# asharakeh/pod_compare

Hardware: AMD Instinct MI355X
Metric: images/sec (BayesOD+MC-dropout, 1280x720) (higher is better)
Workload: dtype f32 (convolutions: every fp32 product from 2-way f16 splits of the power-of-two-scaled fp32 operands, 3 partial products, fp32 accumulate; closer to fp64 than the fp32 MFMA: profiles/r05_f16_split_numerics.txt)

## Files before the change

### include/pod_mi355x.h

```cpp
#ifndef POD_MI355X_H
#define POD_MI355X_H

#include <stddef.h>
#include <stdint.h>

#ifdef __cplusplus
extern "C" {
#endif

#define POD_ABI_VERSION 18
#define POD_MAX_LEVELS 8
#define POD_MAX_CLASSES 16
#define POD_MAX_RUNS 64
#define POD_MAX_TOPK 2048
#define POD_MAX_PROP_SAMPLES 1024
#define POD_MAX_CLS_SAMPLES 64
#define POD_MAX_CANDIDATES 8192
#define POD_MAX_DETECTIONS 128
#define POD_COCO_MAX_IOU 16
#define POD_COCO_MAX_REC 128
#define POD_COCO_MAX_AREA 4
#define POD_COCO_MAX_MAXDET 4
#define POD_COCO_MAX_KEEP 128
#define POD_COCO_LDS_GT 64
// ... 248 lines not shown
    const float* cov;
    const float* probs;
    const float* colours;
    const int32_t* count;
    float* out;
    int32_t* n_out;
    int32_t max_n, box_stride, cov_stride, prob_stride, n_probs, colour_mode, colour_stride;
    int32_t cov_pairing;
    float colour[4];
    int32_t frame_h, frame_w;
    float scale, alpha;
} PodVisList;

typedef struct PodVisFrame {
    const uint8_t* src;
    int64_t sy, sx, sc;
    int32_t src_h, src_w, bgr, bilinear;
    int32_t frame_h, frame_w, out_h, out_w;
    uint8_t* dst;
    float scale, stroke;
    const float* inst[2];
    const int32_t* n_inst[2];
    const float* labels;
    const uint8_t* atlas;
    int32_t n_labels, reserved;
} PodVisFrame;

int pod_vis_layout(const PodVisList* lists, int32_t n_lists, pod_stream_t stream);
int pod_vis_render(const PodVisFrame* frames, int32_t n_frames, pod_stream_t stream);


#define POD_C1_RELU 1
#define POD_C1_RESIDUAL_UP2 2
int64_t pod_conv1x1_filter_split_bytes(int32_t Cout, int32_t Cin);
int pod_conv1x1_filter_split(const float* weight, void* Ws, int32_t Cout, int32_t Cin, pod_stream_t stream);
int pod_reduce_partials(const float* partials, int32_t n_splits, int64_t split_stride, const float* bias, const float* residual, float* y,
                        int64_t n, int32_t Cout, int32_t relu, float* out_amax, pod_stream_t stream);
int pod_conv1x1_split(const float* x, float* y, const void* Ws, const float* bias, const float* residual, int32_t H_out, int32_t W_out,
                      int32_t H_in, int32_t W_in, int32_t stride, int32_t Cin, int32_t Cout, int32_t flags, int32_t n_splits, float* partials,
                      int32_t waves, const float* in_amax, float* out_amax, pod_stream_t stream);

typedef struct PodWorkspace {
    const float* anchors;
    float* mean_cls;  float* mean_cls_var;  float* mean_delta;  float* mean_reg_var;
    uint64_t* cand_keys;  int32_t* cand_count;  uint64_t* maybe_bits;
    uint64_t* sel_keys;   int32_t* sel_count;
    uint64_t* cat_keys;   int32_t* cat_level;
    float* probs_dense;
    int32_t* n_total;     int32_t* cand_anchor_idx;  int32_t* cand_level;  int32_t* cand_class;
    float* cand_score;    float* cand_probs;  float* cand_delta;  float* cand_reg_var;  float* cand_anchor;
    float* cand_run_delta;
    float* boxes;  float* cov;
    int32_t* keep;  int32_t* n_keep;  void* nms_scratch;
    float* m_boxes;  float* m_cov;  float* m_scores;  int32_t* m_classes;  float* m_probs;
    int32_t n_capacity;  int32_t reserved;
} PodWorkspace;

#define POD_MODE_STANDARD_NMS 0
#define POD_MODE_BAYES_OD 1
#define POD_MODE_ANCHOR_STATISTICS 2

int pod_run_image(const PodConfig* cfg, const PodLevel* levels, const PodWorkspace* ws, int32_t mode,
                  int32_t box_merge_mode, int32_t cls_merge_mode, int32_t image_h, int32_t image_w,
                  int32_t out_h, int32_t out_w, const PodDetections* out, pod_stream_t stream);
int pod_run_image_part(const PodConfig* cfg, const PodLevel* levels, const PodWorkspace* ws, int32_t mode,
                  int32_t box_merge_mode, int32_t cls_merge_mode, int32_t image_h, int32_t image_w,
// ... 7 lines not shown
```

### pod_compare_amd/conv1x1.py

```python
from typing import Optional

import torch

from . import amax, hip


class Conv1x1:

    def __init__(self, weight: torch.Tensor, bias: Optional[torch.Tensor], stride: int = 1):
        assert weight.is_cuda and weight.dtype == torch.float32 and weight.dim() == 4 and tuple(weight.shape[2:]) == (1, 1)
        self.K, self.C, self.stride = int(weight.shape[0]), int(weight.shape[1]), int(stride)
        if self.C % 16 or self.K % 64 or self.stride not in (1, 2):
            raise ValueError("pod_conv1x1_split: Cin %% 16 == 0, Cout %% 64 == 0, stride 1 or 2 required, got Cin=%d Cout=%d stride=%d" % (self.C, self.K, self.stride))
        self.Ws = torch.empty(2 * self.K * self.C + 8, dtype=torch.int16, device=weight.device)
        hip.check(hip.load().pod_conv1x1_filter_split(weight.detach().reshape(self.K, self.C).contiguous().data_ptr(), self.Ws.data_ptr(), self.K, self.C,
                                                      hip.current_stream()), "pod_conv1x1_filter_split")
        self.bias = None if bias is None else bias.detach().to(torch.float32).contiguous().clone()

    @staticmethod
    def eligible(conv: Optional[torch.nn.Conv2d]) -> bool:
        return (conv is not None and tuple(conv.kernel_size) == (1, 1) and tuple(conv.padding) == (0, 0) and conv.groups == 1
                and tuple(conv.dilation) == (1, 1) and conv.stride[0] == conv.stride[1] and conv.stride[0] in (1, 2)
                and conv.in_channels % 16 == 0 and conv.out_channels % 64 == 0)

    def out_hw(self, h: int, w: int):
        return ((h - 1) // self.stride + 1, (w - 1) // self.stride + 1)

    def splits_for(self, p_out: int, simds: int = 1024) -> int:
        tiles = ((p_out + 63) // 64) * (self.K // 64)
        nks = self.C // 16
        out_mb = p_out * self.K * 4 / 1e6
        step = 0.38
        best, best_t = 1, (nks // self.auto_waves(tiles, nks)) * step
        for s in (2, 4, 8, 16):
            if nks % s or nks // s < 4 or tiles * s > simds:
                continue
            t = (nks // s // self.auto_waves(tiles * s, nks // s)) * step + 3.0 + (s + 1) * out_mb / 4.0
            if t < best_t:
                best, best_t = s, t
        return best

    @staticmethod
    def auto_waves(tiles: int, per_split: int) -> int:
        waves = 1
        while waves < 4 and per_split % (waves * 4) == 0 and per_split // (waves * 2) >= 8 and tiles * waves * 2 <= 1024:
            waves *= 2
        return waves

    def __call__(self, x: torch.Tensor, h: int, w: int, relu: bool = False, residual: Optional[torch.Tensor] = None,
                 n_splits: Optional[int] = None, waves: int = 0, out: Optional[torch.Tensor] = None, residual_up2: bool = False) -> torch.Tensor:
        assert x.is_cuda and x.dtype == torch.float32 and x.is_contiguous() and tuple(x.shape) == (h * w, self.C)
        ho, wo = self.out_hw(h, w)
        y = torch.empty((ho * wo, self.K), dtype=torch.float32, device=x.device) if out is None else out
        assert y.is_contiguous() and tuple(y.shape) == (ho * wo, self.K) and y.dtype == torch.float32
        s = self.splits_for(ho * wo) if n_splits is None else int(n_splits)
        if residual is not None and residual_up2:
            hr, wr = (ho + 1) // 2, (wo + 1) // 2
            assert residual.is_contiguous() and tuple(residual.shape) == (hr * wr, self.K) and residual.dtype == torch.float32
            if s > 1:
                residual = residual.view(hr, wr, self.K).repeat_interleave(2, 0).repeat_interleave(2, 1)[:ho, :wo].reshape(ho * wo, self.K).contiguous()
                residual_up2 = False
        else:
            residual_up2 = False
        if residual is not None and not residual_up2:
            assert residual.is_contiguous() and tuple(residual.shape) == tuple(y.shape) and residual.dtype == torch.float32
        partials = torch.empty((s, ho * wo, self.K), dtype=torch.float32, device=x.device) if s > 1 else None
        hip.check(hip.load().pod_conv1x1_split(x.data_ptr(), y.data_ptr(), self.Ws.data_ptr(), hip.ptr(self.bias), hip.ptr(residual), ho, wo, h, w, self.stride,
                                               self.C, self.K, (1 if relu else 0) | (2 if residual_up2 else 0), s, hip.ptr(partials), int(waves), amax.of(x).data_ptr(), amax.produced(y).data_ptr(),
                                               hip.current_stream()), "pod_conv1x1_split")
        return y


class Stem7x7:

    def __init__(self, weight: torch.Tensor, bias: Optional[torch.Tensor]):
        assert weight.is_cuda and weight.dtype == torch.float32 and tuple(weight.shape) == (64, 3, 7, 7)
        self.Ws = torch.empty(2 * 64 * 192 + 8, dtype=torch.int16, device=weight.device)
        self._bounds = {}
        hip.check(hip.load().pod_stem7x7_filter_split(weight.detach().contiguous().data_ptr(), self.Ws.data_ptr(), hip.current_stream()), "pod_stem7x7_filter_split")
        self.bias = None if bias is None else bias.detach().to(torch.float32).contiguous().clone()

    @staticmethod
    def eligible(conv: Optional[torch.nn.Conv2d]) -> bool:
        return (conv is not None and tuple(conv.weight.shape) == (64, 3, 7, 7) and tuple(conv.stride) == (2, 2) and tuple(conv.padding) == (3, 3)
                and conv.groups == 1 and tuple(conv.dilation) == (1, 1))

    def __call__(self, x: torch.Tensor, relu: bool = True, mean: Optional[torch.Tensor] = None, std: Optional[torch.Tensor] = None,
                 padded_hw: Optional[tuple] = None):
        assert x.is_cuda and x.dtype in (torch.float32, torch.uint8) and x.is_contiguous() and x.numel() == 3 * x.shape[-2] * x.shape[-1]
        hi, wi = int(x.shape[-2]), int(x.shape[-1])
        h, w = (hi, wi) if padded_hw is None else (int(padded_hw[0]), int(padded_hw[1]))
        assert (mean is None) == (std is None) and h >= hi and w >= wi
        if mean is not None:
            assert mean.is_cuda and std.is_cuda and mean.dtype == std.dtype == torch.float32 and mean.numel() == std.numel() == 3 and mean.is_contiguous() and std.is_contiguous()
        ho, wo = (h - 1) // 2 + 1, (w - 1) // 2 + 1
        y = torch.empty((ho * wo, 64), dtype=torch.float32, device=x.device)
        bound = self._input_bound(x, mean, std)
        hip.check(hip.load().pod_stem7x7_split(x.data_ptr(), 1 if x.dtype == torch.uint8 else 0, hi, wi, hip.ptr(mean), hip.ptr(std), y.data_ptr(), self.Ws.data_ptr(),
                                               hip.ptr(self.bias), h, w, 1 if relu else 0, bound.data_ptr(), amax.produced(y).data_ptr(),
                                               hip.current_stream()), "pod_stem7x7_split")
        return y, ho, wo
# ... 53 lines not shown
```

### pod_compare_amd/csrc/k13_conv1x1_split.hip

```cpp
#include "pod_wino.h"

#ifdef POD_C1_TRACE
static __device__ long long g_c1_trace[8192 * 4];
static __device__ long long g_c1_cycles[8192 * 4];
#define C1_STAMP(k)                                                                                   \
    do {                                                                                              \
        const unsigned wg_ = blockIdx.y * gridDim.x + blockIdx.x;                                     \
        if (threadIdx.x == 0 && wg_ < 8192) {                                                         \
            g_c1_trace[wg_ * 4 + (k)] = wall_clock64();                                               \
            g_c1_cycles[wg_ * 4 + (k)] = clock64();                                                   \
        }                                                                                             \
    } while (0)
#else
#define C1_STAMP(k)
#endif

namespace pod {

typedef uint32_t c1_u32x4 __attribute__((ext_vector_type(4)));
constexpr int C1_KS_U16 = 2 * 2 * 256;
constexpr int C1_TOP = 14;

struct C1Params {
    const float* x;
// ... 160 lines not shown
            }
#pragma unroll
            for (int cb = 0; cb < NCB; ++cb)
#pragma unroll
                for (int q = 0; q < 4; ++q)
                    r[cb][q] = (k0 + 32 * cb + 8 * q < P.Cout) ? *reinterpret_cast<const f32x4*>(res + re0 + 32 * cb + 8 * q) : f32x4{0.f, 0.f, 0.f, 0.f};
        }
#pragma unroll
        for (int cb = 0; cb < NCB; ++cb) {
#pragma unroll
            for (int q = 0; q < 4; ++q) {
                const int k = k0 + 32 * cb + 8 * q;
                if (k >= P.Cout) continue;
                f32x4 v = f32x4{acc[cb][pb][4 * q], acc[cb][pb][4 * q + 1], acc[cb][pb][4 * q + 2], acc[cb][pb][4 * q + 3]};
                v = __builtin_elementwise_fma(v, inv, final_pass && bias ? *reinterpret_cast<const f32x4*>(bias + k) : f32x4{0.f, 0.f, 0.f, 0.f});
                if (final_pass) {
                    if (res) v += r[cb][q];
                    if (P.relu) {
                        v.x = fmaxf(v.x, 0.f); v.y = fmaxf(v.y, 0.f); v.z = fmaxf(v.z, 0.f); v.w = fmaxf(v.w, 0.f);
                    }
                    lmax = fmaxf(fmaxf(lmax, fmaxf(fabsf(v.x), fabsf(v.y))), fmaxf(fabsf(v.z), fabsf(v.w)));
                }
                if (!(POD_C1_ELIM & 8) || v.x == 12345.678f) *reinterpret_cast<f32x4*>(yo + e0 + 32 * cb + 8 * q) = v;
            }
        }
    }
    if (final_pass && P.out_amax) wino_publish_amax(P.out_amax, lmax);
#ifdef POD_C1_TRACE
    __builtin_amdgcn_s_waitcnt(0);
    C1_STAMP(3);
#endif
}

__device__ __forceinline__ void c1_epilogue(const C1Params& P, float* const lds_o, f32x16 (&acc)[2][2], int tp, int tc, int lane, int i32, int h, float sx) {
    constexpr int NCB = 2;
    const float inv1 = wino_pow2_inverse(sx) * wino_pow2_inverse(wino_pow2_scale(*reinterpret_cast<const float*>(P.Ws + (int64_t)P.Cout * P.Cin * 2), C1_TOP));
    const f32x4 inv = f32x4{inv1, inv1, inv1, inv1};
    float lmax = 0.0f;
    float* __restrict__ const yo = P.y + (int64_t)blockIdx.y * P.split_stride;
    const float* __restrict__ const res = P.residual;
    const bool final_pass = P.split_stride == 0;
    const int oc = lane & 15, op = lane >> 4;
    const int gp0 = tp * 64 + op;
    const int64_t e0 = (int64_t)gp0 * P.Cout + tc * 64 + 4 * oc;
    f32x4 r[16];
    if (final_pass && res && P.res_up2) {
        int oy = gp0 / P.W_out, ox = gp0 - oy * P.W_out;
#pragma unroll
        for (int j = 0; j < 16; ++j) {
            r[j] = (gp0 + 4 * j < P.P_out) ? *reinterpret_cast<const f32x4*>(res + ((int64_t)(oy >> 1) * P.W_res + (ox >> 1)) * P.Cout + tc * 64 + 4 * oc)
                                           : f32x4{0.f, 0.f, 0.f, 0.f};
            ox += 4;
            while (ox >= P.W_out) {
                ox -= P.W_out;
                ++oy;
            }
        }
    } else if (final_pass && res) {
#pragma unroll
        for (int j = 0; j < 16; ++j) r[j] = (gp0 + 4 * j < P.P_out) ? *reinterpret_cast<const f32x4*>(res + e0 + (int64_t)(4 * j) * P.Cout) : f32x4{0.f, 0.f, 0.f, 0.f};
    }
    f32x4 b4 = f32x4{0.f, 0.f, 0.f, 0.f};
    if (final_pass && P.bias) b4 = *reinterpret_cast<const f32x4*>(P.bias + tc * 64 + 4 * oc);
#pragma unroll
    for (int pb = 0; pb < 2; ++pb)
#pragma unroll
        for (int cb = 0; cb < NCB; ++cb)
#pragma unroll
            for (int q = 0; q < 4; ++q) {
                const int pix = 32 * pb + i32, c = 8 * cb + 2 * q + h;
                *reinterpret_cast<f32x4*>(lds_o + pix * 64 + 4 * (c ^ (i32 & 15))) =
                    f32x4{acc[cb][pb][4 * q], acc[cb][pb][4 * q + 1], acc[cb][pb][4 * q + 2], acc[cb][pb][4 * q + 3]};
            }
#pragma unroll
    for (int j = 0; j < 16; ++j) {
        const int pix = 4 * j + op;
        f32x4 v = __builtin_elementwise_fma(*reinterpret_cast<const f32x4*>(lds_o + pix * 64 + 4 * (oc ^ (pix & 15))), inv, b4);
        if (final_pass) {
            if (res) v += r[j];
            if (P.relu) {
                v.x = fmaxf(v.x, 0.f); v.y = fmaxf(v.y, 0.f); v.z = fmaxf(v.z, 0.f); v.w = fmaxf(v.w, 0.f);
            }
        }
        if (gp0 + 4 * j < P.P_out) {
            *reinterpret_cast<f32x4*>(yo + e0 + (int64_t)(4 * j) * P.Cout) = v;
            lmax = fmaxf(fmaxf(lmax, fmaxf(fabsf(v.x), fabsf(v.y))), fmaxf(fabsf(v.z), fabsf(v.w)));
        }
    }
    if (final_pass && P.out_amax) wino_publish_amax(P.out_amax, lmax);
}

template <int NCB, int WAVES>
__global__ void __launch_bounds__(64 * WAVES, WAVES > 1 ? 1 : 2) k_conv1x1_split_lds(const C1Params P) {
    __shared__ __attribute__((aligned(16))) float lds_all[WAVES][2][64 * 32];
    const int wave = threadIdx.x >> 6;
    float (*const lds_a)[64 * 32] = lds_all[wave];
    const int lane = threadIdx.x & 63, i32 = lane & 31, h = lane >> 5;
    const int xcd = blockIdx.x & 7, wi = (int)(blockIdx.x >> 3);
    const int tp = (wi / P.n_ct) * 8 + xcd, tc = wi % P.n_ct;
    if (tp >= P.n_pt) return;
    C1_STAMP(0);
    const int nks_all = P.Cin >> 4, nks = P.ks_per_split / WAVES, ks0 = (int)blockIdx.y * P.ks_per_split + wave * nks;
    int32_t soff[8];
#pragma unroll
    for (int j = 0; j < 8; ++j) {
        const int pl = 8 * j + (lane >> 3), p = tp * 64 + pl;
        const int q = p < P.P_out ? p : 0;
        int pin = q;
        if (P.stride != 1) {
            const int oy = q / P.W_out, ox = q - oy * P.W_out;
            pin = (P.stride * oy) * P.W_in + P.stride * ox;
        }
        soff[j] = pin * P.Cin + ks0 * 16 + 4 * ((lane & 7) ^ ((pl >> 1) & 7));
    }
    const float* __restrict__ const xg = P.x;
    const int key = (i32 >> 1) & 7;
    const uint16_t* __restrict__ const wa = P.Ws + ((int64_t)(tc * NCB) * nks_all + ks0) * C1_KS_U16 + (h * 32 + i32) * 8;
    const int64_t w_cb = (int64_t)nks_all * C1_KS_U16;
    const float sx = __builtin_bit_cast(float, __builtin_amdgcn_readfirstlane(__builtin_bit_cast(int, wino_pow2_scale(wino_read_amax(P.in_amax), C1_TOP))));

    f32x16 acc[NCB][2];
#pragma unroll
// ... 76 lines not shown
    for (int j0 = 0; j0 < nks; j0 += 6) trip(trip, c1_ic<0>{}, j0);
    C1_STAMP(2);

    if constexpr (WAVES > 1) {
        if (wave > 0) {
            float* o = &lds_a[0][0];
#pragma unroll
            for (int cb = 0; cb < NCB; ++cb)
#pragma unroll
                for (int pb = 0; pb < 2; ++pb)
#pragma unroll
                    for (int r = 0; r < 16; ++r) o[((cb * 2 + pb) * 16 + r) * 64 + lane] = acc[cb][pb][r];
        }
        __syncthreads();
        if (wave > 0) return;
#pragma unroll
        for (int w = 1; w < WAVES; ++w) {
            const float* o = &lds_all[w][0][0];
#pragma unroll
            for (int cb = 0; cb < NCB; ++cb)
#pragma unroll
                for (int pb = 0; pb < 2; ++pb)
#pragma unroll
                    for (int r = 0; r < 16; ++r) acc[cb][pb][r] += o[((cb * 2 + pb) * 16 + r) * 64 + lane];
        }
    }
    c1_epilogue(P, &lds_a[0][0], acc, tp, tc, lane, i32, h, sx);
#ifdef POD_C1_TRACE
    __builtin_amdgcn_s_waitcnt(0);
    C1_STAMP(3);
#endif
}

__global__ void __launch_bounds__(256) k_conv1x1_reduce(const float* __restrict__ partials, int32_t n_splits, int64_t split_stride, const float* __restrict__ bias,
                                                        const float* __restrict__ residual, float* __restrict__ y, int64_t n4, int32_t Cout, int32_t relu,
                                                        float* __restrict__ out_amax) {
    const int64_t stride = (int64_t)gridDim.x * blockDim.x;
    float lmax = 0.0f;
    for (int64_t i = (int64_t)blockIdx.x * blockDim.x + threadIdx.x; i < n4; i += stride) {
        f32x4 v = *reinterpret_cast<const f32x4*>(partials + 4 * i);
        for (int s = 1; s < n_splits; ++s) v += *reinterpret_cast<const f32x4*>(partials + (int64_t)s * split_stride + 4 * i);
        if (bias) v += *reinterpret_cast<const f32x4*>(bias + (int)((4 * i) % Cout));
        if (residual) v += *reinterpret_cast<const f32x4*>(residual + 4 * i);
        if (relu) {
            v.x = fmaxf(v.x, 0.f); v.y = fmaxf(v.y, 0.f); v.z = fmaxf(v.z, 0.f); v.w = fmaxf(v.w, 0.f);
        }
        *reinterpret_cast<f32x4*>(y + 4 * i) = v;
        lmax = fmaxf(fmaxf(lmax, fmaxf(fabsf(v.x), fabsf(v.y))), fmaxf(fabsf(v.z), fabsf(v.w)));
    }
    if (out_amax) wino_publish_amax_block(out_amax, lmax);
}

}

extern "C" int64_t pod_conv1x1_filter_split_bytes(int32_t Cout, int32_t Cin) {
    if (Cout < 32 || (Cout & 31) != 0 || Cin < 16 || (Cin & 15) != 0) return 0;
    return (int64_t)Cout * Cin * 4 + 16;
}

extern "C" int pod_conv1x1_filter_split(const float* weight, void* Ws, int32_t Cout, int32_t Cin, pod_stream_t stream) {
    if (!weight || !Ws || Cout < 32 || (Cout & 31) != 0 || Cin < 16 || (Cin & 15) != 0 || (reinterpret_cast<uintptr_t>(Ws) & 15u) != 0) return POD_E_INVALID;
    const int64_t n = (int64_t)Cout * (Cin / 2);
    float* amax = reinterpret_cast<float*>(reinterpret_cast<char*>(Ws) + (int64_t)Cout * Cin * 4);
    if (hipMemsetAsync(amax, 0, 16, (hipStream_t)stream) != hipSuccess) return POD_E_LAUNCH;
    hipLaunchKernelGGL(pod::k_conv1x1_filter_amax, dim3(256), dim3(256), 0, (hipStream_t)stream, weight, (int64_t)Cout * Cin, amax);
    POD_CHECK_LAUNCH();
    hipLaunchKernelGGL(pod::k_conv1x1_filter_split, dim3((unsigned)((n + 255) / 256)), dim3(256), 0, (hipStream_t)stream, weight, reinterpret_cast<uint16_t*>(Ws), amax,
                       Cout, Cin);
    POD_CHECK_LAUNCH();
    return POD_OK;
}

extern "C" int pod_conv1x1_split(const float* x, float* y, const void* Ws, const float* bias, const float* residual, int32_t H_out, int32_t W_out, int32_t H_in,
                                 int32_t W_in, int32_t stride, int32_t Cin, int32_t Cout, int32_t flags, int32_t n_splits, float* partials, int32_t waves,
                                 const float* in_amax, float* out_amax, pod_stream_t stream) {
    if (!x || !y || !Ws || !in_amax || x == y || H_out < 1 || W_out < 1 || (stride != 1 && stride != 2) || Cin < 16 || (Cin & 15) != 0 || Cout < 64 || (Cout & 63) != 0)
        return POD_E_INVALID;
    if (H_in < (H_out - 1) * stride + 1 || W_in < (W_out - 1) * stride + 1 || (stride == 1 && (H_in != H_out || W_in != W_out))) return POD_E_INVALID;
    const int64_t P_out = (int64_t)H_out * W_out;
    if (P_out * (Cout > Cin ? Cout : Cin) >= ((int64_t)1 << 31) || (int64_t)H_in * W_in * Cin >= ((int64_t)1 << 31)) return POD_E_INVALID;
    const int nks = Cin / 16;
    if (n_splits < 1 || n_splits > 16 || nks % n_splits != 0 || (n_splits > 1 && !partials)) return POD_E_INVALID;
    const int res_up2 = (flags & POD_C1_RESIDUAL_UP2) ? 1 : 0, relu = flags & POD_C1_RELU;
    if (res_up2 && (!residual || n_splits > 1)) return POD_E_INVALID;
    if (waves < 0 || waves > 4 || waves == 3) return POD_E_INVALID;
    {
        const int per_split = nks / n_splits;
        if (waves == 0) {
            const int64_t tiles = ((P_out + 63) / 64) * (Cout / 64) * n_splits;
            waves = 1;
            while (waves < 4 && per_split % (waves * 4) == 0 && per_split / (waves * 2) >= 8 && tiles * waves * 2 <= 1024) waves *= 2;
        }
        if (waves > 1 && (per_split % (2 * waves) != 0)) return POD_E_INVALID;
    }
    if (((reinterpret_cast<uintptr_t>(x) | reinterpret_cast<uintptr_t>(y) | reinterpret_cast<uintptr_t>(Ws) | reinterpret_cast<uintptr_t>(bias) |
          reinterpret_cast<uintptr_t>(residual) | reinterpret_cast<uintptr_t>(partials)) & 15u) != 0 ||
        ((reinterpret_cast<uintptr_t>(in_amax) | reinterpret_cast<uintptr_t>(out_amax)) & 3u) != 0)
        return POD_E_INVALID;
    pod::C1Params P;
    P.x = x; P.y = n_splits > 1 ? partials : y; P.Ws = reinterpret_cast<const uint16_t*>(Ws); P.bias = bias; P.residual = residual;
    P.in_amax = in_amax; P.out_amax = out_amax;
    P.P_out = (int32_t)P_out; P.W_out = W_out; P.W_in = W_in; P.stride = stride; P.Cin = Cin; P.Cout = Cout; P.relu = relu;
    P.res_up2 = res_up2; P.W_res = (W_out + 1) / 2;
    P.n_pt = (int32_t)((P_out + 63) / 64); P.n_ct = Cout / 64;
    P.ks_per_split = nks / n_splits;
    P.split_stride = n_splits > 1 ? P_out * Cout : 0;
    const int64_t grid = 8LL * ((P.n_pt + 7) / 8) * P.n_ct;
    if (grid > 0x7FFFFFFFLL) return POD_E_INVALID;
    if (POD_C1_DIRECT)
        hipLaunchKernelGGL((pod::k_conv1x1_split<2, POD_C1_RING>), dim3((unsigned)grid, (unsigned)n_splits), dim3(64), 0, (hipStream_t)stream, P);
    else if ((P.ks_per_split & 1) == 0 && waves == 4)
        hipLaunchKernelGGL((pod::k_conv1x1_split_lds<2, 4>), dim3((unsigned)grid, (unsigned)n_splits), dim3(256), 0, (hipStream_t)stream, P);
    else if ((P.ks_per_split & 1) == 0 && waves == 2)
        hipLaunchKernelGGL((pod::k_conv1x1_split_lds<2, 2>), dim3((unsigned)grid, (unsigned)n_splits), dim3(128), 0, (hipStream_t)stream, P);
    else if ((P.ks_per_split & 1) == 0)
        hipLaunchKernelGGL((pod::k_conv1x1_split_lds<2, 1>), dim3((unsigned)grid, (unsigned)n_splits), dim3(64), 0, (hipStream_t)stream, P);
    else
        hipLaunchKernelGGL((pod::k_conv1x1_split<2, POD_C1_RING>), dim3((unsigned)grid, (unsigned)n_splits), dim3(64), 0, (hipStream_t)stream, P);
    POD_CHECK_LAUNCH();
    if (n_splits > 1) {
        const int64_t n4 = P_out * Cout / 4;
        int64_t blocks = (n4 + 255) / 256;
        if (blocks > 2048) blocks = 2048;
        hipLaunchKernelGGL(pod::k_conv1x1_reduce, dim3((unsigned)blocks), dim3(256), 0, (hipStream_t)stream, partials, n_splits, P_out * Cout, bias, residual, y, n4,
                           Cout, relu, out_amax);
        POD_CHECK_LAUNCH();
    }
    return POD_OK;
}

extern "C" int pod_reduce_partials(const float* partials, int32_t n_splits, int64_t split_stride, const float* bias, const float* residual, float* y, int64_t n,
                                   int32_t Cout, int32_t relu, float* out_amax, pod_stream_t stream) {
    if (!partials || !y || n_splits < 1 || n_splits > 16 || n < 0 || (n & 3) != 0 || Cout < 4 || (Cout & 3) != 0 || n % Cout != 0) return POD_E_INVALID;
    if (n_splits > 1 && (split_stride < n || (split_stride & 3) != 0)) return POD_E_INVALID;
    if (((reinterpret_cast<uintptr_t>(partials) | reinterpret_cast<uintptr_t>(y) | reinterpret_cast<uintptr_t>(bias) | reinterpret_cast<uintptr_t>(residual)) & 15u) != 0)
        return POD_E_INVALID;
    if (n == 0) return POD_OK;
    int64_t blocks = (n / 4 + 255) / 256;
    if (blocks > 4096) blocks = 4096;
    hipLaunchKernelGGL(pod::k_conv1x1_reduce, dim3((unsigned)blocks), dim3(256), 0, (hipStream_t)stream, partials, n_splits, split_stride, bias, residual, y, n / 4,
                       Cout, relu, out_amax);
    POD_CHECK_LAUNCH();
// ... 39 lines not shown
```

### pod_compare_amd/hip.py

```python
import ctypes
import os
from ctypes import POINTER, Structure, c_double, c_float, c_int32, c_int64, c_size_t, c_uint64, c_void_p
from typing import Optional

import torch

from .build import LIB

POD_ABI_VERSION = 18
POD_MAX_LEVELS = 8
POD_MAX_CLASSES = 16
POD_MAX_RUNS = 64
POD_MAX_TOPK = 2048
POD_MAX_PROP_SAMPLES = 1024
POD_MAX_CLS_SAMPLES = 64
POD_MAX_CANDIDATES = 8192
POD_MAX_DETECTIONS = 128
POD_COCO_MAX_IOU, POD_COCO_MAX_REC, POD_COCO_MAX_AREA, POD_COCO_MAX_MAXDET, POD_COCO_MAX_KEEP, POD_COCO_LDS_GT = 16, 128, 4, 4, 128, 64
POD_CALIB_MAX_EDGES, POD_CALIB_BLOCK = 15, 1024
POD_VIS_MAX_INSTANCES, POD_VIS_INST_WORDS, POD_VIS_PRIM_WORDS, POD_VIS_LAUNCH_FRAMES = 256, 32, 12, 8
POD_VIS_COLOUR_ENTROPY, POD_VIS_COLOUR_FIXED, POD_VIS_COLOUR_PALETTE, POD_VIS_COLOUR_ARRAY = 0, 1, 2, 3
POD_VIS_COV_BY_RANK, POD_VIS_COV_OWN = 0, 1
POD_VIS_LABEL_BOX, POD_VIS_LABEL_GLYPH = 3, 4

EXPORTS = ("pod_abi_version", "pod_mc_merge_score", "pod_maybe_words", "pod_score_maybe", "pod_merge_score_fused", "pod_reset_counters", "pod_level_topk", "pod_gather_candidates", "pod_gather_decode",
           "pod_decode_cov", "pod_nms_scratch_bytes", "pod_nms_cluster", "pod_bayes_fuse", "pod_anchor_stats_merge",
           "pod_ensemble_append", "pod_ensemble_merge",
           "pod_finalize", "pod_reg_nll", "pod_relu_dropout", "pod_bias_act", "pod_bias_act_to_nchw", "pod_bias_act_to_nhwc", "pod_expand_dropout", "pod_match_groundtruth", "pod_run_image", "pod_run_image_part",
           "pod_absmax", "pod_wino_filter_transform", "pod_wino_conv3x3", "pod_wino_filter_split_bytes", "pod_wino_filter_transform_split", "pod_wino_conv3x3_split", "pod_sparse_reach", "pod_sparse_live_blocks", "pod_wino_reduce", "pod_conv1x1_filter_split_bytes", "pod_conv1x1_filter_split", "pod_conv1x1_split", "pod_reduce_partials", "pod_stem7x7_filter_split", "pod_stem7x7_split", "pod_maxpool3x3s2_cl", "pod_im2col3x3s2_cl",
           "pod_coco_eval_scratch_bytes", "pod_coco_eval_images", "pod_coco_accumulate_workspace_bytes", "pod_coco_accumulate",
           "pod_calib_keys", "pod_calib_reg_counts", "pod_calib_min_uncertainty_workspace_bytes", "pod_calib_min_uncertainty",
           "pod_calib_marginal_sort_workspace_bytes", "pod_calib_marginal_sort", "pod_calib_marginal_bins", "pod_calib_marginal_error_workspace_bytes",
           "pod_calib_marginal_error", "pod_vis_layout", "pod_vis_render")
_SIZE_QUERIES = ("pod_abi_version", "pod_nms_scratch_bytes", "pod_coco_eval_scratch_bytes", "pod_coco_accumulate_workspace_bytes", "pod_maybe_words",
                 "pod_wino_filter_split_bytes", "pod_conv1x1_filter_split_bytes", "pod_calib_min_uncertainty_workspace_bytes",
                 "pod_calib_marginal_sort_workspace_bytes", "pod_calib_marginal_error_workspace_bytes")
TEST_EXPORTS = ("pod_dump_cls_normals", "pod_dump_box_normals", "pod_debug_f16_split2")
POD_MODE_STANDARD_NMS, POD_MODE_BAYES_OD, POD_MODE_ANCHOR_STATISTICS = 0, 1, 2


class PodLevel(Structure):
    _fields_ = [("cls", c_void_p), ("cls_var", c_void_p), ("delta", c_void_p), ("reg_var", c_void_p), ("eps_cls", c_void_p),
# ... 174 lines not shown
```

### pod_compare_amd/torch_ops.py

```python
from typing import List, Tuple

import torch

from . import hip, hotpath

_LIB = torch.library.Library("pod_mi355x", "DEF")
_LIB.define("predict(Tensor[] box_cls, Tensor[] box_delta, Tensor[] box_cls_var, Tensor[] box_reg_var, Tensor[] anchors, "
            "str mode, int[] image_size, int[] out_size, int num_classes=7, int topk_candidates=1000, float score_thresh=0.05, "
            "float nms_thresh=0.5, int max_detections=100, int cls_var_num_samples=10, float affinity_thresh=0.9, "
            "bool merge_quirk=True, str box_merge_mode='bayesian_inference', str cls_merge_mode='max_score', int draw_id=-1) "
            "-> (Tensor, Tensor, Tensor, Tensor, Tensor)")
_LIB.define("nms_cluster(Tensor boxes, Tensor scores, Tensor classes, float nms_thresh, int max_detections, int num_classes) -> Tensor")
_LIB.define("reg_nll(Tensor means, Tensor covs, Tensor gt) -> Tensor")
_LIB.define("wino_filter_transform(Tensor weight) -> Tensor")
_LIB.define("wino_conv3x3(Tensor src, Tensor U, Tensor? bias, Tensor blocks, int K, int out_elements, bool planes=False, bool relu=False, "
            "float dropout_p=0.0, int seed=0, int offset=0) -> Tensor")
_LIB.define("conv1x1_filter_split(Tensor weight) -> Tensor")
_LIB.define("conv1x1_split(Tensor x, Tensor Ws, Tensor? bias, Tensor? residual, int h, int w, int stride, int cout, bool relu=False, int n_splits=1) -> Tensor")
_LIB.define("stem7x7_filter_split(Tensor weight) -> Tensor")
_LIB.define("stem7x7_split(Tensor frame, Tensor Ws, Tensor? bias, Tensor? mean, Tensor? std, int padded_h, int padded_w, bool relu=True) -> Tensor")
_LIB.define("maxpool3x3s2_cl(Tensor x, int h, int w) -> Tensor")
_LIB.define("im2col3x3s2_cl(Tensor x, int h, int w, bool relu=False) -> Tensor")

_PATHS = {}
_MAX_PATHS = 16
_TABLES_OK = {}


def _check_dense(name: str, ts: List[torch.Tensor], like: List[torch.Tensor]) -> None:
    torch._check(len(ts) == len(like), lambda: "{}: {} levels, box_cls has {}".format(name, len(ts), len(like)))
    for l, (t, ref) in enumerate(zip(ts, like)):
        torch._check(t.is_cuda and t.dtype == torch.float32 and t.dim() == 4, lambda: "{}[{}] must be a CUDA fp32 (runs, A*C, H, W) tensor".format(name, l))
        torch._check(t.shape[0] == ref.shape[0] and tuple(t.shape[2:]) == tuple(ref.shape[2:]) and t.device == ref.device,
                     lambda: "{}[{}]: shape {} does not match box_cls {}".format(name, l, tuple(t.shape), tuple(ref.shape)))


def _predict(box_cls, box_delta, box_cls_var, box_reg_var, anchors, mode, image_size, out_size, num_classes=7, topk_candidates=1000,
             score_thresh=0.05, nms_thresh=0.5, max_detections=100, cls_var_num_samples=10, affinity_thresh=0.9, merge_quirk=True,
             box_merge_mode="bayesian_inference", cls_merge_mode="max_score", draw_id=-1) -> Tuple[torch.Tensor, ...]:
    torch._check(len(box_cls) >= 1, lambda: "box_cls: at least one FPN level")
    _check_dense("box_cls", box_cls, box_cls)
    _check_dense("box_delta", box_delta, box_cls)
    if box_cls_var:
        _check_dense("box_cls_var", box_cls_var, box_cls)
    if box_reg_var:
        _check_dense("box_reg_var", box_reg_var, box_cls)
    torch._check(len(anchors) == len(box_cls) and len(image_size) == 2 and len(out_size) == 2, lambda: "anchors per level; (h, w) sizes")
    K = int(num_classes)
    torch._check(box_cls[0].shape[1] % K == 0, lambda: "box_cls channels {} are not A * num_classes".format(box_cls[0].shape[1]))
    A = box_cls[0].shape[1] // K
    n_runs = int(box_cls[0].shape[0])
# ... 94 lines not shown
              & (last_out * per_px <= int(out_elements)) & (((w >> 12) & 0xFFF) * 16 < ((n + gcols - 1) // gcols) * (H + 1))
              & ((w & 0xFFF) * 16 < gcols * (W + 1)) & (n * H * W * max(C, per_px) * 4 <= 2 ** 31 - 256))
        torch._check(bool(ok.all()), lambda: "blocks: a record lies outside src / the output / the 32-bit canvas (record {})".format(int((~ok).nonzero()[0])))
        if len(_TABLES_OK) >= 64:
            _TABLES_OK.pop(next(iter(_TABLES_OK)))
        _TABLES_OK[tkey] = blocks
    out = torch.zeros(int(out_elements), dtype=torch.float32, device=src.device) if planes else \
        torch.empty((src.shape[0], Kpad), dtype=torch.float32, device=src.device)
    with torch.cuda.device(src.device):
        hip.check(hip.load().pod_wino_conv3x3(hip.ptr(src), hip.ptr(out), hip.ptr(U), hip.ptr(bias), hip.ptr(blocks), int(blocks.shape[0]), C, Kpad,
                                              int(K) if planes else 0, 1 if relu else 0, float(dropout_p), int(seed), int(offset),
                                              None, hip.current_stream()), "pod_wino_conv3x3")
    return out


def _absmax_word(t: torch.Tensor) -> torch.Tensor:
    w = torch.zeros(512, dtype=torch.float32, device=t.device)
    with torch.cuda.device(t.device):
        hip.check(hip.load().pod_absmax(hip.ptr(t), t.numel(), hip.ptr(w), hip.current_stream()), "pod_absmax")
    return w


def _conv1x1_filter_split(weight) -> torch.Tensor:
    torch._check(weight.is_cuda and weight.dtype == torch.float32 and weight.dim() in (2, 4) and weight.numel() == weight.shape[0] * weight.shape[1],
                 lambda: "weight: CUDA fp32 (Cout, Cin) or (Cout, Cin, 1, 1)")
    cout, cin = int(weight.shape[0]), int(weight.shape[1])
    torch._check(cout >= 64 and cout % 64 == 0 and cin >= 16 and cin % 16 == 0, lambda: "Cout % 64 == 0 and Cin % 16 == 0 required")
    ws = torch.empty(2 * cout * cin + 8, dtype=torch.int16, device=weight.device)
    with torch.cuda.device(weight.device):
        hip.check(hip.load().pod_conv1x1_filter_split(hip.ptr(weight.contiguous()), hip.ptr(ws), cout, cin, hip.current_stream()), "pod_conv1x1_filter_split")
    return ws


def _conv1x1_split(x, Ws, bias, residual, h, w, stride, cout, relu=False, n_splits=1) -> torch.Tensor:
    torch._check(x.is_cuda and x.dtype == torch.float32 and x.dim() == 2 and x.is_contiguous() and x.shape[0] == h * w, lambda: "x: contiguous CUDA fp32 (h * w, Cin)")
    cin = int(x.shape[1])
    torch._check(stride in (1, 2) and cout >= 64 and cout % 64 == 0 and cin >= 16 and cin % 16 == 0, lambda: "stride 1 or 2, cout % 64 == 0, Cin % 16 == 0")
    torch._check(Ws.is_cuda and Ws.dtype == torch.int16 and Ws.numel() == 2 * cout * cin + 8, lambda: "Ws: conv1x1_filter_split of a (cout, Cin) weight")
    ho, wo = (h - 1) // stride + 1, (w - 1) // stride + 1
    torch._check(bias is None or (bias.is_cuda and bias.dtype == torch.float32 and bias.numel() == cout and bias.is_contiguous()), lambda: "bias: cout fp32 values")
    torch._check(residual is None or (residual.is_cuda and residual.dtype == torch.float32 and residual.is_contiguous() and tuple(residual.shape) == (ho * wo, cout)),
                 lambda: "residual: contiguous (h_out * w_out, cout) fp32")
    nks = cin // 16
    torch._check(1 <= n_splits <= 16 and nks % n_splits == 0, lambda: "n_splits must divide Cin / 16 (1 .. 16)")
    y = torch.empty((ho * wo, cout), dtype=torch.float32, device=x.device)
    partials = torch.empty((n_splits, ho * wo, cout), dtype=torch.float32, device=x.device) if n_splits > 1 else None
    with torch.cuda.device(x.device):
        hip.check(hip.load().pod_conv1x1_split(hip.ptr(x), hip.ptr(y), hip.ptr(Ws), hip.ptr(bias), hip.ptr(residual), ho, wo, int(h), int(w), int(stride), cin, int(cout),
                                               1 if relu else 0, int(n_splits), hip.ptr(partials), 0, hip.ptr(_absmax_word(x)), None, hip.current_stream()), "pod_conv1x1_split")
    return y


def _stem7x7_filter_split(weight) -> torch.Tensor:
    torch._check(weight.is_cuda and weight.dtype == torch.float32 and tuple(weight.shape) == (64, 3, 7, 7), lambda: "weight: CUDA fp32 (64, 3, 7, 7)")
    ws = torch.empty(2 * 64 * 192 + 8, dtype=torch.int16, device=weight.device)
    with torch.cuda.device(weight.device):
        hip.check(hip.load().pod_stem7x7_filter_split(hip.ptr(weight.contiguous()), hip.ptr(ws), hip.current_stream()), "pod_stem7x7_filter_split")
    return ws


def _stem7x7_split(frame, Ws, bias, mean, std, padded_h, padded_w, relu=True) -> torch.Tensor:
    torch._check(frame.is_cuda and frame.dtype in (torch.uint8, torch.float32) and frame.dim() == 3 and frame.shape[0] == 3 and frame.is_contiguous(),
                 lambda: "frame: contiguous CUDA uint8 / fp32 (3, H, W)")
    hi, wi = int(frame.shape[1]), int(frame.shape[2])
    torch._check(padded_h >= hi and padded_w >= wi and padded_h <= 16384 and padded_w <= 16384, lambda: "padded extent must contain the frame (<= 16384)")
    torch._check(Ws.is_cuda and Ws.dtype == torch.int16 and Ws.numel() == 2 * 64 * 192 + 8, lambda: "Ws: stem7x7_filter_split of the (64, 3, 7, 7) weight")
    torch._check((mean is None) == (std is None), lambda: "mean and std: both or neither")
    for t in (mean, std):
        torch._check(t is None or (t.is_cuda and t.dtype == torch.float32 and t.numel() == 3 and t.is_contiguous()), lambda: "mean / std: 3 contiguous CUDA fp32 values")
    torch._check(bias is None or (bias.is_cuda and bias.dtype == torch.float32 and bias.numel() == 64 and bias.is_contiguous()), lambda: "bias: 64 fp32 values")
    ho, wo = (int(padded_h) - 1) // 2 + 1, (int(padded_w) - 1) // 2 + 1
    y = torch.empty((ho * wo, 64), dtype=torch.float32, device=frame.device)
    bound = torch.full((512,), 255.0, dtype=torch.float32, device=frame.device) if frame.dtype == torch.uint8 else _absmax_word(frame)
    if mean is not None:
        bound = (bound + mean.abs().max()) / std.abs().min()
    with torch.cuda.device(frame.device):
        hip.check(hip.load().pod_stem7x7_split(hip.ptr(frame), 1 if frame.dtype == torch.uint8 else 0, hi, wi, hip.ptr(mean), hip.ptr(std), hip.ptr(y), hip.ptr(Ws),
                                               hip.ptr(bias), int(padded_h), int(padded_w), 1 if relu else 0, hip.ptr(bound), None, hip.current_stream()), "pod_stem7x7_split")
    return y


def _maxpool3x3s2_cl(x, h, w) -> torch.Tensor:
# ... 30 lines not shown
```

Baseline: 131.4.

## Add wide 128x128 tile conv1x1 kernel with four waves sharing LDS

Adds a conv1x1 kernel in which four waves cooperatively stage a 128-pixel by 128-channel tile of activations and split filters into double-buffered LDS. Each wave computes a 64x64 sub-tile. It is enabled by default for layers with Cout%128==0, Cin%32==0 and channel counts between 128 and 2048, and it replaces split-K for those layers. The aim is better operand reuse and less global traffic per MFMA, plus no partial-sum reduction pass. The cost is fewer workgroups on small spatial layers and more LDS per block.

Measured after the change: 131.0. About the same (-0.3%).

```diff
diff --git a/include/pod_mi355x.h b/include/pod_mi355x.h
--- a/include/pod_mi355x.h
+++ b/include/pod_mi355x.h
@@ -304,6 +304,7 @@
 
 #define POD_C1_RELU 1
 #define POD_C1_RESIDUAL_UP2 2
+#define POD_C1_WIDE 4
 int64_t pod_conv1x1_filter_split_bytes(int32_t Cout, int32_t Cin);
 int pod_conv1x1_filter_split(const float* weight, void* Ws, int32_t Cout, int32_t Cin, pod_stream_t stream);
 int pod_reduce_partials(const float* partials, int32_t n_splits, int64_t split_stride, const float* bias, const float* residual, float* y,
diff --git a/pod_compare_amd/conv1x1.py b/pod_compare_amd/conv1x1.py
--- a/pod_compare_amd/conv1x1.py
+++ b/pod_compare_amd/conv1x1.py
@@ -1,8 +1,18 @@
+import os
 from typing import Optional
 
 import torch
 
 from . import amax, hip
+
+
+def _wide_pixels(spec: str):
+    lo, _, hi = spec.partition(":")
+    return (int(lo) if lo else 0, int(hi) if hi else 1 << 62)
+
+
+_WIDE_ENV = os.environ.get("POD_C1_WIDE", "1")
+_WIDE_PIXELS = _wide_pixels(os.environ.get("POD_C1_WIDE_PIXELS", ""))
 
 
 class Conv1x1:
@@ -40,6 +50,11 @@
                 best, best_t = s, t
         return best
 
+    def wide_for(self, p_out: int) -> bool:
+        if _WIDE_ENV == "0" or self.K % 128 or self.C % 32 or min(self.C, self.K) < 128 or self.C > 2048:
+            return False
+        return _WIDE_PIXELS[0] <= p_out <= _WIDE_PIXELS[1]
+
     @staticmethod
     def auto_waves(tiles: int, per_split: int) -> int:
         waves = 1
@@ -48,12 +63,15 @@
         return waves
 
     def __call__(self, x: torch.Tensor, h: int, w: int, relu: bool = False, residual: Optional[torch.Tensor] = None,
-                 n_splits: Optional[int] = None, waves: int = 0, out: Optional[torch.Tensor] = None, residual_up2: bool = False) -> torch.Tensor:
+                 n_splits: Optional[int] = None, waves: int = 0, out: Optional[torch.Tensor] = None, residual_up2: bool = False,
+                 wide: Optional[bool] = None) -> torch.Tensor:
         assert x.is_cuda and x.dtype == torch.float32 and x.is_contiguous() and tuple(x.shape) == (h * w, self.C)
         ho, wo = self.out_hw(h, w)
         y = torch.empty((ho * wo, self.K), dtype=torch.float32, device=x.device) if out is None else out
         assert y.is_contiguous() and tuple(y.shape) == (ho * wo, self.K) and y.dtype == torch.float32
-        s = self.splits_for(ho * wo) if n_splits is None else int(n_splits)
+        if wide is None:
+            wide = n_splits is None and waves == 0 and self.wide_for(ho * wo)
+        s = 1 if wide and n_splits is None else self.splits_for(ho * wo) if n_splits is None else int(n_splits)
         if residual is not None and residual_up2:
             hr, wr = (ho + 1) // 2, (wo + 1) // 2
             assert residual.is_contiguous() and tuple(residual.shape) == (hr * wr, self.K) and residual.dtype == torch.float32
@@ -66,7 +84,7 @@
             assert residual.is_contiguous() and tuple(residual.shape) == tuple(y.shape) and residual.dtype == torch.float32
         partials = torch.empty((s, ho * wo, self.K), dtype=torch.float32, device=x.device) if s > 1 else None
         hip.check(hip.load().pod_conv1x1_split(x.data_ptr(), y.data_ptr(), self.Ws.data_ptr(), hip.ptr(self.bias), hip.ptr(residual), ho, wo, h, w, self.stride,
-                                               self.C, self.K, (1 if relu else 0) | (2 if residual_up2 else 0), s, hip.ptr(partials), int(waves), amax.of(x).data_ptr(), amax.produced(y).data_ptr(),
+                                               self.C, self.K, (1 if relu else 0) | (2 if residual_up2 else 0) | (hip.POD_C1_WIDE if wide else 0), s, hip.ptr(partials), int(waves), amax.of(x).data_ptr(), amax.produced(y).data_ptr(),
                                                hip.current_stream()), "pod_conv1x1_split")
         return y
 
diff --git a/pod_compare_amd/csrc/k13_conv1x1_split.hip b/pod_compare_amd/csrc/k13_conv1x1_split.hip
--- a/pod_compare_amd/csrc/k13_conv1x1_split.hip
+++ b/pod_compare_amd/csrc/k13_conv1x1_split.hip
@@ -216,7 +216,8 @@
 #endif
 }
 
-__device__ __forceinline__ void c1_epilogue(const C1Params& P, float* const lds_o, f32x16 (&acc)[2][2], int tp, int tc, int lane, int i32, int h, float sx) {
+__device__ __forceinline__ void c1_epilogue(const C1Params& P, float* const lds_o, f32x16 (&acc)[2][2], int tp, int tc, int lane, int i32, int h, float sx,
+                                            int amax_slot = -1) {
     constexpr int NCB = 2;
     const float inv1 = wino_pow2_inverse(sx) * wino_pow2_inverse(wino_pow2_scale(*reinterpret_cast<const float*>(P.Ws + (int64_t)P.Cout * P.Cin * 2), C1_TOP));
     const f32x4 inv = f32x4{inv1, inv1, inv1, inv1};
@@ -271,7 +272,12 @@
             lmax = fmaxf(fmaxf(lmax, fmaxf(fabsf(v.x), fabsf(v.y))), fmaxf(fabsf(v.z), fabsf(v.w)));
         }
     }
-    if (final_pass && P.out_amax) wino_publish_amax(P.out_amax, lmax);
+    if (final_pass && P.out_amax) {
+        if (amax_slot < 0)
+            wino_publish_amax(P.out_amax, lmax);
+        else
+            wino_publish_amax1(P.out_amax + amax_slot * POD_AMAX_STRIDE, lmax);
+    }
 }
 
 template <int NCB, int WAVES>
@@ -414,6 +420,116 @@
 #endif
 }
 
+__global__ void __launch_bounds__(256) k_conv1x1_split_wide(const C1Params P) {
+    constexpr int NCB = 2;
+    __shared__ __attribute__((aligned(16))) float lds[4 * 4096];
+    const int wave = threadIdx.x >> 6, pi = wave & 1, cj = wave >> 1;
+    const int lane = threadIdx.x & 63, i32 = lane & 31, h = lane >> 5;
+    const int xcd = blockIdx.x & 7, wi = (int)(blockIdx.x >> 3);
+    const int tp = (wi / P.n_ct) * 8 + xcd, tc = wi % P.n_ct;
+    if (tp >= P.n_pt) return;
+    const int nks_all = P.Cin >> 4, npairs = nks_all >> 1;
+    int32_t soff[4];
+#pragma unroll
+    for (int j = 0; j < 4; ++j) {
+        const int pl = 32 * wave + 8 * j + (lane >> 3), p = tp * 128 + pl;
+        const int q = p < P.P_out ? p : 0;
+        int pin = q;
+        if (P.stride != 1) {
+            const int oy = q / P.W_out, ox = q - oy * P.W_out;
+            pin = (P.stride * oy) * P.W_in + P.stride * ox;
+        }
+        soff[j] = pin * P.Cin + 4 * ((lane & 7) ^ ((pl >> 1) & 7));
+    }
+    const float* __restrict__ const xg = P.x;
+    const uint16_t* __restrict__ const wsrc = P.Ws + ((int64_t)(tc * 4 + wave) * nks_all) * C1_KS_U16 + lane * 8;
+    float* const xw = lds + (32 * wave) * 32 + lane * 4;
+    c1_u32x4* const fw = reinterpret_cast<c1_u32x4*>(lds + 8192) + (wave * 4) * 64 + lane;
+    const float* const xr = lds + (pi * 64 + i32) * 32;
+    const c1_u32x4* const fr = reinterpret_cast<const c1_u32x4*>(lds + 8192) + (2 * cj * 4) * 64 + lane;
+    const int key = (i32 >> 1) & 7;
+    const float sx = __builtin_bit_cast(float, __builtin_amdgcn_readfirstlane(__builtin_bit_cast(int, wino_pow2_scale(wino_read_amax(P.in_amax), C1_TOP))));
+
+    f32x16 acc[NCB][2];
+#pragma unroll
+    for (int cb = 0; cb < NCB; ++cb)
+#pragma unroll
+        for (int pb = 0; pb < 2; ++pb)
+#pragma unroll
+            for (int r = 0; r < 16; ++r) acc[cb][pb][r] = 0.f;
+    f32x4 stg[4];
+    c1_u32x4 wst[4];
+    auto stage_load = [&](int pair) __attribute__((always_inline)) {
+#pragma unroll
+        for (int j = 0; j < 4; ++j) stg[j] = *reinterpret_cast<const f32x4*>(xg + soff[j] + pair * 32);
+#pragma unroll
+        for (int i = 0; i < 4; ++i) wst[i] = *reinterpret_cast<const c1_u32x4*>(wsrc + (int64_t)pair * (2 * C1_KS_U16) + i * 512);
+    };
+    auto stage_write = [&](auto b_t) __attribute__((always_inline)) {
+        constexpr int b = decltype(b_t)::value;
+#pragma unroll
+        for (int j = 0; j < 4; ++j) *reinterpret_cast<f32x4*>(xw + b * 4096 + j * 256) = stg[j];
+#pragma unroll
+        for (int i = 0; i < 4; ++i) fw[b * 1024 + i * 64] = wst[i];
+    };
+    auto step = [&](auto t_t, auto b_t) __attribute__((always_inline)) {
+        constexpr int t = decltype(t_t)::value;
+        constexpr int b = decltype(b_t)::value;
+        c1_u32x4 wf[NCB][2];
+#pragma unroll
+        for (int cb = 0; cb < NCB; ++cb)
+#pragma unroll
+            for (int term = 0; term < 2; ++term) wf[cb][term] = fr[b * 1024 + (cb * 4 + 2 * t + term) * 64];
+        c1_u32x4 at[2][2];
+#pragma unroll
+        for (int pb = 0; pb < 2; ++pb) {
+            const float* row = xr + b * 4096 + pb * 1024;
+            const f32x4 a0 = *reinterpret_cast<const f32x4*>(row + 4 * ((4 * t + 2 * h) ^ key));
+            const f32x4 a1 = *reinterpret_cast<const f32x4*>(row + 4 * ((4 * t + 2 * h + 1) ^ key));
+#pragma unroll
+            for (int i = 0; i < 4; ++i) {
+                float lo = i < 2 ? a0[2 * (i & 1)] : a1[2 * (i & 1)], hi = i < 2 ? a0[2 * (i & 1) + 1] : a1[2 * (i & 1) + 1];
+                const uint32_t t0 = wino_f16_pair_scaled(lo, hi, sx);
+                wino_f16_residual_scaled(t0, lo, hi, sx);
+                at[pb][0][i] = t0;
+                at[pb][1][i] = wino_f16_pair(lo, hi);
+            }
+        }
+#pragma unroll
+        for (int prod = 0; prod < 3; ++prod) {
+            const int sa = prod == 1 ? 1 : 0;
+            const int sb = prod == 0 ? 1 : 0;
+#pragma unroll
+            for (int cb = 0; cb < NCB; ++cb)
+#pragma unroll
+                for (int pb = 0; pb < 2; ++pb)
+                    acc[cb][pb] = __builtin_amdgcn_mfma_f32_32x32x16_f16(__builtin_bit_cast(wino_f16x8, wf[cb][sa]), __builtin_bit_cast(wino_f16x8, at[pb][sb]), acc[cb][pb], 0, 0, 0);
+        }
+    };
+    auto pair_body = [&](int pair, auto b_t) __attribute__((always_inline)) {
+        constexpr int b = decltype(b_t)::value;
+        step(c1_ic<0>{}, b_t);
+        step(c1_ic<1>{}, b_t);
+        if (pair + 1 < npairs) {
+            stage_write(c1_ic<b ^ 1>{});
+            __syncthreads();
+            if (pair + 2 < npairs) stage_load(pair + 2);
+        }
+    };
+    stage_load(0);
+    stage_write(c1_ic<0>{});
+    __syncthreads();
+    if (npairs > 1) stage_load(1);
+    for (int pair = 0; pair < npairs; pair += 2) {
+        pair_body(pair, c1_ic<0>{});
+        if (pair + 1 < npairs) pair_body(pair + 1, c1_ic<1>{});
+    }
+    __syncthreads();
+    const int tp64 = tp * 2 + pi, tc64 = tc * 2 + cj;
+    const int slot = (((tp64 >> 3) * (P.n_ct * 2) + tc64) & 1) * 8 + (tp64 & 7);
+    c1_epilogue(P, lds + wave * 4096, acc, tp64, tc64, lane, i32, h, sx, slot);
+}
+
 __global__ void __launch_bounds__(256) k_conv1x1_reduce(const float* __restrict__ partials, int32_t n_splits, int64_t split_stride, const float* __restrict__ bias,
                                                         const float* __restrict__ residual, float* __restrict__ y, int64_t n4, int32_t Cout, int32_t relu,
                                                         float* __restrict__ out_amax) {
@@ -463,8 +579,10 @@
     if (P_out * (Cout > Cin ? Cout : Cin) >= ((int64_t)1 << 31) || (int64_t)H_in * W_in * Cin >= ((int64_t)1 << 31)) return POD_E_INVALID;
     const int nks = Cin / 16;
     if (n_splits < 1 || n_splits > 16 || nks % n_splits != 0 || (n_splits > 1 && !partials)) return POD_E_INVALID;
-    const int res_up2 = (flags & POD_C1_RESIDUAL_UP2) ? 1 : 0, relu = flags & POD_C1_RELU;
+    const int res_up2 = (flags & POD_C1_RESIDUAL_UP2) ? 1 : 0, relu = flags & POD_C1_RELU, wide = (flags & POD_C1_WIDE) ? 1 : 0;
+    if (flags & ~(POD_C1_RELU | POD_C1_RESIDUAL_UP2 | POD_C1_WIDE)) return POD_E_INVALID;
     if (res_up2 && (!residual || n_splits > 1)) return POD_E_INVALID;
+    if (wide && (n_splits != 1 || waves > 1 || (Cout & 127) != 0 || (Cin & 31) != 0)) return POD_E_INVALID;
     if (waves < 0 || waves > 4 || waves == 3) return POD_E_INVALID;
     {
         const int per_split = nks / n_splits;
@@ -487,9 +605,14 @@
     P.n_pt = (int32_t)((P_out + 63) / 64); P.n_ct = Cout / 64;
     P.ks_per_split = nks / n_splits;
     P.split_stride = n_splits > 1 ? P_out * Cout : 0;
+    if (wide) {
+        P.n_pt = (int32_t)((P_out + 127) / 128); P.n_ct = Cout / 128;
+    }
     const int64_t grid = 8LL * ((P.n_pt + 7) / 8) * P.n_ct;
     if (grid > 0x7FFFFFFFLL) return POD_E_INVALID;
-    if (POD_C1_DIRECT)
+    if (wide)
+        hipLaunchKernelGGL(pod::k_conv1x1_split_wide, dim3((unsigned)grid), dim3(256), 0, (hipStream_t)stream, P);
+    else if (POD_C1_DIRECT)
         hipLaunchKernelGGL((pod::k_conv1x1_split<2, POD_C1_RING>), dim3((unsigned)grid, (unsigned)n_splits), dim3(64), 0, (hipStream_t)stream, P);
     else if ((P.ks_per_split & 1) == 0 && waves == 4)
         hipLaunchKernelGGL((pod::k_conv1x1_split_lds<2, 4>), dim3((unsigned)grid, (unsigned)n_splits), dim3(256), 0, (hipStream_t)stream, P);
diff --git a/pod_compare_amd/hip.py b/pod_compare_amd/hip.py
--- a/pod_compare_amd/hip.py
+++ b/pod_compare_amd/hip.py
@@ -8,6 +8,7 @@
 from .build import LIB
 
 POD_ABI_VERSION = 18
+POD_C1_RELU, POD_C1_RESIDUAL_UP2, POD_C1_WIDE = 1, 2, 4
 POD_MAX_LEVELS = 8
 POD_MAX_CLASSES = 16
 POD_MAX_RUNS = 64
diff --git a/pod_compare_amd/torch_ops.py b/pod_compare_amd/torch_ops.py
--- a/pod_compare_amd/torch_ops.py
+++ b/pod_compare_amd/torch_ops.py
@@ -16,7 +16,7 @@
 _LIB.define("wino_conv3x3(Tensor src, Tensor U, Tensor? bias, Tensor blocks, int K, int out_elements, bool planes=False, bool relu=False, "
             "float dropout_p=0.0, int seed=0, int offset=0) -> Tensor")
 _LIB.define("conv1x1_filter_split(Tensor weight) -> Tensor")
-_LIB.define("conv1x1_split(Tensor x, Tensor Ws, Tensor? bias, Tensor? residual, int h, int w, int stride, int cout, bool relu=False, int n_splits=1) -> Tensor")
+_LIB.define("conv1x1_split(Tensor x, Tensor Ws, Tensor? bias, Tensor? residual, int h, int w, int stride, int cout, bool relu=False, int n_splits=1, bool wide=False) -> Tensor")
 _LIB.define("stem7x7_filter_split(Tensor weight) -> Tensor")
 _LIB.define("stem7x7_split(Tensor frame, Tensor Ws, Tensor? bias, Tensor? mean, Tensor? std, int padded_h, int padded_w, bool relu=True) -> Tensor")
 _LIB.define("maxpool3x3s2_cl(Tensor x, int h, int w) -> Tensor")
@@ -177,7 +177,7 @@
     return ws
 
 
-def _conv1x1_split(x, Ws, bias, residual, h, w, stride, cout, relu=False, n_splits=1) -> torch.Tensor:
+def _conv1x1_split(x, Ws, bias, residual, h, w, stride, cout, relu=False, n_splits=1, wide=False) -> torch.Tensor:
     torch._check(x.is_cuda and x.dtype == torch.float32 and x.dim() == 2 and x.is_contiguous() and x.shape[0] == h * w, lambda: "x: contiguous CUDA fp32 (h * w, Cin)")
     cin = int(x.shape[1])
     torch._check(stride in (1, 2) and cout >= 64 and cout % 64 == 0 and cin >= 16 and cin % 16 == 0, lambda: "stride 1 or 2, cout % 64 == 0, Cin % 16 == 0")
@@ -188,11 +188,12 @@
                  lambda: "residual: contiguous (h_out * w_out, cout) fp32")
     nks = cin // 16
     torch._check(1 <= n_splits <= 16 and nks % n_splits == 0, lambda: "n_splits must divide Cin / 16 (1 .. 16)")
+    torch._check(not wide or (cout % 128 == 0 and cin % 32 == 0 and n_splits == 1), lambda: "wide: cout % 128 == 0, Cin % 32 == 0, n_splits == 1")
     y = torch.empty((ho * wo, cout), dtype=torch.float32, device=x.device)
     partials = torch.empty((n_splits, ho * wo, cout), dtype=torch.float32, device=x.device) if n_splits > 1 else None
     with torch.cuda.device(x.device):
         hip.check(hip.load().pod_conv1x1_split(hip.ptr(x), hip.ptr(y), hip.ptr(Ws), hip.ptr(bias), hip.ptr(residual), ho, wo, int(h), int(w), int(stride), cin, int(cout),
-                                               1 if relu else 0, int(n_splits), hip.ptr(partials), 0, hip.ptr(_absmax_word(x)), None, hip.current_stream()), "pod_conv1x1_split")
+                                               (1 if relu else 0) | (hip.POD_C1_WIDE if wide else 0), int(n_splits), hip.ptr(partials), 0, hip.ptr(_absmax_word(x)), None, hip.current_stream()), "pod_conv1x1_split")
     return y
 
 
```
